# thu-ml/zhusuan

Hardware: NVIDIA B200
Metric: leapfrog-steps*chains/sec (higher is better)
Workload: dtype f32

## Files before the change

include/zsb200.h:

```cpp
#ifndef ZSB200_H_
#define ZSB200_H_
#include <stddef.h>
#include <stdint.h>

#ifdef __cplusplus
extern "C" {
#endif

#define ZSB_OK 0
#define ZSB_ERR_INVALID (-1)
#define ZSB_ERR_CUDA (-2)
#define ZSB_ERR_UNSUPPORTED (-3)

int zsb_version(void);
int zsb_last_error(char* buf, size_t n);
int zsb_device_count(void);
int zsb_stream_sync(void* stream);
int zsb_random_set_device_epoch(const uint32_t* epoch);
int zsb_random_bump_epoch(uint32_t* epoch, uint32_t by, void* stream);

enum {
  ZSB_HMC_STATE_T = 0, ZSB_HMC_STATE_STEP_SIZE = 1, ZSB_HMC_STATE_TUNER_STEP = 2,
  ZSB_HMC_STATE_LOG_EPS_BAR = 3, ZSB_HMC_STATE_H_BAR = 4, ZSB_HMC_STATE_MU = 5,
  ZSB_HMC_STATE_EWMV_T = 6, ZSB_HMC_STATE_EPS_USED = 7, ZSB_HMC_STATE_ACC_MEAN = 8,
// ... 153 lines not shown
                               int64_t D, int impl, void* stream);
int zsb_hmc_dense_tc_config(int bk);
int zsb_hmc_dense_split_lo_f32(const float* q, float* lo, int64_t n, void* stream);
int zsb_hmc_dense_h16_prepare_f32(const float* q, void* planes, float* scales, int64_t n,
                                  void* stream);
int zsb_hmc_dense_leapfrog_h16_f32(const float* q_cur, const void* q_cur_planes, float* q_next,
                                   void* q_next_planes, const float* p_in, float* p_out,
                                   const void* P_h16, const void* P_l16, const float* scales,
                                   const float* bvec, const float* mu, const float* mass,
                                   const float* state, float p_scale, float* lp_part,
                                   float* k_part, int64_t chains, int64_t D, void* stream);
int zsb_hmc_dense_h16i_prepare_f32(const float* q, float* scales, int64_t n, void* stream);
int zsb_hmc_dense_leapfrog_h16i_f32(const float* q_cur, float* q_next, const float* p_in,
                                    float* p_out, const void* P_h16, const void* P_l16,
                                    float* scales, int pass_index, const float* bvec,
                                    const float* mu, const float* mass, const float* state,
                                    float p_scale, float* lp_part, float* k_part, int64_t chains,
                                    int64_t D, void* stream);
int zsb_hmc_dense_trajectory_h16_f32(const float* q0, const void* planes0, float* qa,
                                     void* planes_a, float* qb, void* planes_b, const float* p0,
                                     float* pw, const void* P_h16, const void* P_l16,
                                     const float* scales, const float* bvec, const float* mu,
                                     const float* mass, const float* state, float* lp0_part,
                                     float* lp1_part, float* k_part, int64_t chains, int64_t D,
                                     int n_leapfrogs, void* stream);
int zsb_hmc_dense_resident_flags(int64_t chains);
int zsb_hmc_dense_resident_group(int64_t D);
int zsb_hmc_dense_resident_h16_f32(void* planes0, void* planes1, const float* p0, float* pw,
                                   const void* P_h16, const void* P_l16, const float* scales,
                                   const float* bvec, const float* mu, const float* mass,
                                   const float* state, float* lp0_part, float* lp1_part,
                                   float* k_part, int32_t* flags, int64_t chains, int64_t D,
                                   int n_leapfrogs, void* stream);
int zsb_hmc_dense_select_planes_f32(float* q, const void* planes, const float* scales,
                                    const int32_t* accept, int64_t chains, int64_t D,
                                    void* stream);
int zsb_hmc_dense_finish_f32(const float* lp_part, const float* k_part, int ntiles, int64_t chains,
                             float const_term, float* lp_out, float* k_out, void* stream);

int zsb_sample_categorical_i32(const float* logits, int64_t logit_rows, int64_t rows,
                               int64_t n_categories, int64_t n_samples, const float* u,
                               uint64_t seed, uint32_t iter, int32_t* out, void* stream);
int zsb_sample_dirichlet_f32(const float* alpha, int64_t alpha_rows, int64_t n_rows,
                             int64_t n_categories, const float* gammas, uint64_t seed,
                             uint32_t iter, float* out, void* stream);
int zsb_sample_gamma_f32(const float* alpha, int64_t alpha_rows, const float* beta,
                         int64_t beta_rows, int64_t n_rows, int64_t row_len, uint64_t seed,
                         uint32_t iter, float* out, void* stream);
int zsb_sample_base_noise_f32(int kind, float* out, int64_t n, uint64_t seed, uint32_t iter,
                              void* stream);
int zsb_sample_count_i32(int kind, const float* param, int64_t param_n, int64_t n_experiments,
                         const float* u, uint64_t seed, uint32_t iter, int32_t* out, int64_t n,
                         void* stream);

int zsb_lntm_phi_t_f32(const float* beta, int64_t n_topics, int64_t n_vocab, float* phi_t,
                       void* stream);
int zsb_lntm_logjoint_f32(const float* eta, const float* eta_mean, const float* eta_logstd,
                          const float* phi_t, const int64_t* doc_ptr, const int32_t* word_idx,
                          const float* word_cnt, float* lp_out, float* grad_out, int64_t chains,
                          int64_t docs, int64_t n_topics, void* stream);

int zsb_sgmcmc_parts(void);
int zsb_sgmcmc_sgld_f32(float* q, const float* g, const float* noise, float lr, int64_t chains,
                        int64_t row_len, uint64_t seed, uint32_t iter, int64_t row0,
                        void* stream);
int zsb_sgmcmc_psgld_f32(float* q, float* aux, const float* g, const float* noise, float lr,
// ... 36 lines not shown
```

zhusuan_b200/csrc/hmc_dense.cu:

```cuda
#include "common.cuh"

namespace {

constexpr int BM = 128, BN = 128, BK = 16;
constexpr int APAD = 4;


__global__ void __launch_bounds__(256, 2)
dense_leapfrog_simt_kernel(const float* __restrict__ q_cur, float* __restrict__ q_next,
                           const float* __restrict__ p_in, float* __restrict__ p_out,
                           const float* __restrict__ P, const float* __restrict__ bvec,
                           const float* __restrict__ mu, const float* __restrict__ mass,
                           const float* __restrict__ state, float p_scale,
                           float* __restrict__ lp_part, float* __restrict__ k_part,
                           int64_t chains, int D) {
  __shared__ __align__(16) float As[2][BK][BM + APAD];
  __shared__ __align__(16) float Bs[2][BK][BN];

  const int tid = threadIdx.x;
  const int tx = tid & 15, ty = tid >> 4;
  const int64_t m0 = (int64_t)blockIdx.y * BM;
  const int n0 = blockIdx.x * BN;

  const int a_row = tid >> 2;
// ... 136 lines not shown
int zsb_dense_split_lo_launch(const float* q, float* lo, int64_t n, cudaStream_t st);
int zsb_dense_tc_ntiles(int D);
int zsb_dense_tc_set_bk(int bk);
int zsb_dense_leapfrog_h16_launch(const float* q_cur, const void* q_cur_planes, float* q_next,
                                  void* q_next_planes, const float* p_in, float* p_out,
                                  const void* P_h16, const void* P_l16, const float* scales,
                                  const float* bvec, const float* mu, const float* mass,
                                  const float* state, float p_scale, float* lp_part, float* k_part,
                                  int64_t chains, int D, cudaStream_t st);
int zsb_dense_h16_prepare_launch(const float* q, void* planes, float* scales, int64_t n,
                                 cudaStream_t st);
int zsb_dense_leapfrog_h16i_launch(const float* q_cur, float* q_next, const float* p_in,
                                   float* p_out, const void* P_h16, const void* P_l16,
                                   float* scales, int pass_index, const float* bvec,
                                   const float* mu, const float* mass, const float* state,
                                   float p_scale, float* lp_part, float* k_part, int64_t chains,
                                   int D, cudaStream_t st);
int zsb_dense_h16i_prepare_launch(const float* q, float* scales, int64_t n, cudaStream_t st);
int zsb_dense_traj_h16_launch(const float* q0, const void* planes0, float* qa, void* planes_a,
                              float* qb, void* planes_b, const float* p0, float* pw,
                              const void* P_h16, const void* P_l16, const float* scales,
                              const float* bvec, const float* mu, const float* mass,
                              const float* state, float* lp0_part, float* lp1_part,
                              float* k_part, int64_t chains, int D, int L, cudaStream_t st);
int zsb_dense_res_h16_launch(void* planes0, void* planes1, const float* p0, float* pw,
                             const void* P_h16, const void* P_l16, const float* scales,
                             const float* bvec, const float* mu, const float* mass,
                             const float* state, float* lp0_part, float* lp1_part, float* k_part,
                             int* flags, int64_t chains, int D, int L, cudaStream_t st);
int zsb_dense_select_planes_launch(float* q, const void* planes, const float* scales,
                                   const int32_t* accept, int64_t chains, int64_t D,
                                   cudaStream_t st);
int zsb_dense_res_group_blocks(int D);

extern "C" {

int zsb_hmc_dense_ntiles(int64_t D, int impl) {
  if (impl == 1) return zsb_dense_tc_ntiles((int)D);
  return (int)zsb_ceil_div(D, BN);
}

int zsb_hmc_dense_leapfrog_f32(const float* q_cur, const float* q_cur_lo, float* q_next,
                               float* q_next_lo, const float* p_in, float* p_out,
                               const float* P, const float* P_lo, const float* bvec,
                               const float* mu, const float* mass, const float* state,
                               float p_scale, float* lp_part, float* k_part, int64_t chains,
                               int64_t D, int impl, void* stream) {
  ZSB_REQUIRE(q_cur && p_in && p_out && P && mass && state, "zsb_hmc_dense_leapfrog_f32: null arg");
  ZSB_REQUIRE(chains > 0 && D > 0 && D % BK == 0 && D <= (1 << 20),
              "zsb_hmc_dense_leapfrog_f32: D must be a positive multiple of 16");
  ZSB_REQUIRE(q_next != q_cur, "zsb_hmc_dense_leapfrog_f32: q_next must not alias q_cur");
  cudaStream_t st = (cudaStream_t)stream;
  if (impl == 1) {
    ZSB_REQUIRE(P_lo && q_cur_lo, "zsb_hmc_dense_leapfrog_f32: impl 1 needs the P_lo / q_lo splits");
    return zsb_dense_leapfrog_tc_launch(q_cur, q_cur_lo, q_next, q_next_lo, p_in, p_out, P, P_lo,
                                        bvec, mu, mass, state, p_scale, lp_part, k_part, chains,
                                        (int)D, st);
  }
  ZSB_REQUIRE(impl == 0, "zsb_hmc_dense_leapfrog_f32: unknown impl %d", impl);
  dim3 grid((unsigned)zsb_ceil_div(D, BN), (unsigned)zsb_ceil_div(chains, BM));
  dense_leapfrog_simt_kernel<<<grid, 256, 0, st>>>(q_cur, q_next, p_in, p_out, P, bvec, mu, mass,
                                                   state, p_scale, lp_part, k_part, chains, (int)D);
  return zsb_check_launch("hmc_dense_leapfrog_simt");
}

int zsb_hmc_dense_tc_config(int bk) {
// ... 45 lines not shown
}

int zsb_hmc_dense_trajectory_h16_f32(const float* q0, const void* planes0, float* qa,
                                     void* planes_a, float* qb, void* planes_b, const float* p0,
                                     float* pw, const void* P_h16, const void* P_l16,
                                     const float* scales, const float* bvec, const float* mu,
                                     const float* mass, const float* state, float* lp0_part,
                                     float* lp1_part, float* k_part, int64_t chains, int64_t D,
                                     int n_leapfrogs, void* stream) {
  ZSB_REQUIRE(q0 && planes0 && qa && planes_a && qb && planes_b && p0 && pw && P_h16 && P_l16 &&
                  scales && mass && state && lp0_part && lp1_part && k_part,
              "zsb_hmc_dense_trajectory_h16_f32: null arg");
  return zsb_dense_traj_h16_launch(q0, planes0, qa, planes_a, qb, planes_b, p0, pw, P_h16, P_l16,
                                   scales, bvec, mu, mass, state, lp0_part, lp1_part, k_part,
                                   chains, (int)D, n_leapfrogs, (cudaStream_t)stream);
}

int zsb_hmc_dense_resident_flags(int64_t chains) { return 2 * (int)zsb_ceil_div(chains, 256); }
int zsb_hmc_dense_resident_group(int64_t D) { return zsb_dense_res_group_blocks((int)D); }
int zsb_hmc_dense_resident_h16_f32(void* planes0, void* planes1, const float* p0, float* pw,
                                   const void* P_h16, const void* P_l16, const float* scales,
                                   const float* bvec, const float* mu, const float* mass,
                                   const float* state, float* lp0_part, float* lp1_part,
                                   float* k_part, int32_t* flags, int64_t chains, int64_t D,
                                   int n_leapfrogs, void* stream) {
  ZSB_REQUIRE(planes0 && planes1 && p0 && pw && P_h16 && P_l16 && scales && mass && state &&
                  lp0_part && lp1_part && k_part && flags,
              "zsb_hmc_dense_resident_h16_f32: null arg");
  ZSB_REQUIRE(p0 != pw, "zsb_hmc_dense_resident_h16_f32: aliased buffers");
  return zsb_dense_res_h16_launch(planes0, planes1, p0, pw, P_h16, P_l16, scales, bvec, mu, mass,
                                  state, lp0_part, lp1_part, k_part, flags, chains, (int)D,
                                  n_leapfrogs, (cudaStream_t)stream);
}
int zsb_hmc_dense_select_planes_f32(float* q, const void* planes, const float* scales,
                                    const int32_t* accept, int64_t chains, int64_t D,
                                    void* stream) {
  ZSB_REQUIRE(q && planes && scales && accept && chains > 0 && D > 0 && D % 2 == 0,
              "zsb_hmc_dense_select_planes_f32: bad args");
  return zsb_dense_select_planes_launch(q, planes, scales, accept, chains, D,
                                        (cudaStream_t)stream);
}

int zsb_hmc_dense_finish_f32(const float* lp_part, const float* k_part, int ntiles, int64_t chains,
                             float const_term, float* lp_out, float* k_out, void* stream) {
  ZSB_REQUIRE(chains > 0 && ntiles > 0, "zsb_hmc_dense_finish_f32: bad sizes");
  int64_t blocks = zsb_ceil_div(chains, 256);
  if (blocks > ZSB_NUM_SMS * 8) blocks = ZSB_NUM_SMS * 8;
  dense_finish_kernel<<<(unsigned)blocks, 256, 0, (cudaStream_t)stream>>>(
      lp_part, k_part, ntiles, chains, const_term, lp_out, k_out);
  return zsb_check_launch("hmc_dense_finish");
}

}
```

zhusuan_b200/csrc/hmc_dense_res.cu:

```cuda
#include "tc_common.cuh"

namespace {

using CR = Cfg2<32>;

struct ResMaps {
  CUtensorMap p_hi, p_lo;
  CUtensorMap q_hi[2], q_lo[2];
};

__device__ __forceinline__ int flag_load_acquire(const int* f) {
  int v;
  asm volatile("ld.acquire.gpu.global.s32 %0, [%1];" : "=r"(v) : "l"(f) : "memory");
  return v;
}
__device__ __forceinline__ void flag_add_release(int* f, int v) {
  asm volatile("red.release.gpu.global.add.s32 [%0], %1;" ::"l"(f), "r"(v) : "memory");
}
__device__ __forceinline__ void flag_wait(const int* f, int target) {
  if (flag_load_acquire(f) >= target) return;
  const long long t0 = clock64();
  while (flag_load_acquire(f) < target) {
    __nanosleep(64);
    if (clock64() - t0 > WAIT_TIMEOUT_CYCLES) {
      printf("zsb dense_res: flag wait timeout (block %d thread %d target %d have %d)\n",
             blockIdx.x, threadIdx.x, target, flag_load_acquire(f));
      __trap();
    }
  }
}

__device__ __forceinline__ void tma_load_2d_2sm_mc(uint32_t dst, const CUtensorMap* map,
                                                   uint32_t bar, int c0, int c1, uint16_t mask) {
  asm volatile(
      "cp.async.bulk.tensor.2d.cta_group::2.shared::cluster.global.mbarrier::complete_tx::bytes"
      ".multicast::cluster [%0], [%1, {%4, %5}], [%2], %3;"
      ::"r"(dst), "l"(map), "r"(bar & PEER_BIT_MASK), "h"(mask), "r"(c0), "r"(c1)
      : "memory");
}
__device__ __forceinline__ void umma_commit_mask(uint32_t bar, uint16_t mask) {
  asm volatile(
      "tcgen05.commit.cta_group::2.mbarrier::arrive::one.shared::cluster.multicast::cluster.b64"
      " [%0], %1;"
      ::"r"(bar), "h"(mask) : "memory");
}

struct ResEpi {
  const __half* __restrict__ hi_cur; const __half* __restrict__ lo_cur;
  __half* __restrict__ hi_nxt; __half* __restrict__ lo_nxt;
  const float* __restrict__ p_in; float* __restrict__ p_out;
  float* __restrict__ lp_part; float* __restrict__ k_part;
  int64_t chains; int D;
  float sq, inv_sq, acc_scale;
};

template <int MODE, int NEXT, int DC>
__device__ __forceinline__ void epilogue_planes(const ResEpi& a, uint32_t trow, int n, bool n_ok,
                                                bool parts_ok, int64_t c0, int64_t part_row,
                                                int lane, float s2, float eps_over_m_sq,
                                                float inv_m, float b_n, float mu_n, bool skip) {
  constexpr int NCOL = BN / 2;
  const uint32_t D = DC ? (uint32_t)DC : (uint32_t)a.D;
  const int64_t chains = a.chains;
  const bool warp_n_ok = __all_sync(0xffffffffu, n_ok);
  const bool fast_tile = warp_n_ok && (c0 + NCOL <= chains) && !skip;
  const int64_t off_t = c0 * (int64_t)D + n;
  const float* __restrict__ pin0 = a.p_in + off_t;
  float* __restrict__ po0 = a.p_out + off_t;
  const unsigned short* __restrict__ hc0 =
      reinterpret_cast<const unsigned short*>(a.hi_cur) + off_t;
  const unsigned short* __restrict__ lc0 =
      reinterpret_cast<const unsigned short*>(a.lo_cur) + off_t;
  __half* __restrict__ hn0 = NEXT ? a.hi_nxt + off_t : nullptr;
  __half* __restrict__ ln0 = NEXT ? a.lo_nxt + off_t : nullptr;

  auto element = [&](float acc, float p, uint32_t hl, float& pn, float& lpv, float& kv,
                     __half& hh, __half& ll) {
    const float Q = __half2float(__ushort_as_half((unsigned short)(hl & 0xFFFFu))) +
                    __half2float(__ushort_as_half((unsigned short)(hl >> 16)));
    const float g = b_n - a.acc_scale * acc;
    pn = fmaf(s2, g, p);
    if (MODE >= 1) lpv = (Q * a.inv_sq - mu_n) * g;
    if (MODE >= 2) kv = pn * pn * inv_m;
    if (NEXT) {
      const float Qn = fmaf(eps_over_m_sq, pn, Q);
      hh = __float2half_rn(Qn);
      ll = __float2half_rn(Qn - __half2float(hh));
    }
  };

  if (fast_tile) {
    auto load = [&](float* pe, uint32_t* he, int c) {
      const size_t cb = (size_t)c * D;
#pragma unroll
      for (int j = 0; j < 16; ++j) {
        pe[j] = __ldcg(pin0 + cb + (uint32_t)j * D);
        const uint32_t h = __ldcg(hc0 + cb + (uint32_t)j * D);
        const uint32_t l = __ldcg(lc0 + cb + (uint32_t)j * D);
        he[j] = h | (l << 16);
      }
    };
    auto compute = [&](const uint32_t* v, const float* pe, const uint32_t* he, int c) {
      const size_t cb = (size_t)c * D;
      float lpv[MODE >= 1 ? 16 : 1], kv[MODE >= 2 ? 16 : 1];
#pragma unroll
      for (int j = 0; j < 16; ++j) {
        float pn, lp1 = 0.f, k1 = 0.f;
        __half hh, ll;
        element(__uint_as_float(v[j]), pe[j], he[j], pn, lp1, k1, hh, ll);
        po0[cb + (uint32_t)j * D] = pn;
        if (MODE >= 1) lpv[j] = lp1;
        if (MODE >= 2) kv[j] = k1;
        if (NEXT) {
          hn0[cb + (uint32_t)j * D] = hh;
          ln0[cb + (uint32_t)j * D] = ll;
        }
      }
      if (MODE >= 1) {
        const float sum = warp_transpose_sum16(lpv, lane);
        if (lane < 16) a.lp_part[part_row + c0 + c + lane] = sum;
      }
      if (MODE >= 2) {
        const float sum = warp_transpose_sum16(kv, lane);
        if (lane < 16) a.k_part[part_row + c0 + c + lane] = sum;
      }
    };
    float pa[16], pb[16];
    uint32_t ha[16], hb[16], va[16], vb[16];
    load(pa, ha, 0);
    tmem_ld16(trow, va);
#pragma unroll 1
    for (int c = 0; c < NCOL; c += 32) {
      load(pb, hb, c + 16);
      tmem_ld_wait();
      tmem_ld16(trow + (uint32_t)(c + 16), vb);
      compute(va, pa, ha, c);
      if (c + 32 < NCOL) load(pa, ha, c + 32);
      tmem_ld_wait();
      if (c + 32 < NCOL) tmem_ld16(trow + (uint32_t)(c + 32), va);
      compute(vb, pb, hb, c + 16);
    }
  } else {
#pragma unroll 1
    for (int c = 0; c < NCOL; c += 16) {
      uint32_t v[16];
      tmem_ld16(trow + (uint32_t)c, v);
      tmem_ld_wait();
      const int64_t cbase = c0 + c;
      if (cbase < chains && !skip) {
        const size_t cb = (size_t)c * D;
        float lpv[MODE >= 1 ? 16 : 1], kv[MODE >= 2 ? 16 : 1];
#pragma unroll
        for (int j = 0; j < 16; ++j) {
          const bool ok = n_ok && cbase + j < chains;
          float p = 0.f;
          uint32_t hl = 0u;
          if (ok) {
            p = __ldcg(pin0 + cb + (uint32_t)j * D);
            hl = (uint32_t)__ldcg(hc0 + cb + (uint32_t)j * D) |
                 ((uint32_t)__ldcg(lc0 + cb + (uint32_t)j * D) << 16);
          }
          float pn, lp1 = 0.f, k1 = 0.f;
          __half hh, ll;
          element(__uint_as_float(v[j]), p, hl, pn, lp1, k1, hh, ll);
          if (MODE >= 1) lpv[j] = ok ? lp1 : 0.f;
          if (MODE >= 2) kv[j] = ok ? k1 : 0.f;
          if (ok) {
            po0[cb + (uint32_t)j * D] = pn;
            if (NEXT) {
              hn0[cb + (uint32_t)j * D] = hh;
              ln0[cb + (uint32_t)j * D] = ll;
            }
          }
        }
        if (MODE >= 1) {
          const float sum = warp_transpose_sum16(lpv, lane);
          if (parts_ok && lane < 16 && cbase + lane < chains)
            a.lp_part[part_row + cbase + lane] = sum;
        }
        if (MODE >= 2) {
          const float sum = warp_transpose_sum16(kv, lane);
          if (parts_ok && lane < 16 && cbase + lane < chains)
            a.k_part[part_row + cbase + lane] = sum;
        }
      }
    }
  }
}

template <int DC, int MC>
__global__ void __launch_bounds__(NUM_THREADS, 1)
dense_res_kernel(const __grid_constant__ ResMaps maps, __half* __restrict__ planes0,
                 __half* __restrict__ planes1, const float* __restrict__ p0,
                 float* __restrict__ pw, const float* __restrict__ bvec,
                 const float* __restrict__ mu, const float* __restrict__ mass,
                 const float* __restrict__ state, float* __restrict__ lp0_part,
                 float* __restrict__ lp1_part, float* __restrict__ k_part, int64_t chains,
                 int D_rt, int L, const float* __restrict__ scales, int* __restrict__ flags,
                 int group_blocks, int dbg, int inplace) {
  using C = CR;
  const int D = DC ? DC : D_rt;
  extern __shared__ uint8_t smem_raw[];
  const uint32_t smem_base = (smem_u32(smem_raw) + 1023u) & ~1023u;
  const uint32_t bars = smem_base + C::STAGES * C::STAGE;
  const uint32_t full_bar = bars;
  const uint32_t empty_bar = bars + 8 * C::STAGES;
  const uint32_t tfull_bar = bars + 16 * C::STAGES;
  const uint32_t tempty_bar = bars + 16 * C::STAGES + 16;
  const uint32_t tmem_slot = bars + 16 * C::STAGES + 32;
  uint32_t* tmem_slot_ptr =
      reinterpret_cast<uint32_t*>(smem_raw + (tmem_slot - smem_u32(smem_raw)));

  const int warp = __shfl_sync(0xffffffffu, (int)(threadIdx.x >> 5), 0);
  const int lane = threadIdx.x & 31;
  const uint32_t crank = cluster_ctarank();
  const uint32_t rank = crank & 1u;
  const uint32_t pidx = crank >> 1;
  const uint32_t leader_rank = crank & ~1u;
  const bool leader = rank == 0;
  const uint16_t pair_mask = (uint16_t)(3u << leader_rank);
  const int n_blk = (D + BM - 1) / BM;
  const int n_pair = (n_blk + 1) / 2;
  const int64_t c_blk = (chains + BN - 1) / BN;
  constexpr int CL = MC ? 4 : 2;
  const int64_t my = blockIdx.x / CL, n_clusters = gridDim.x / CL;
  const int n_kb = D / 64;
  const int flag_per_pass = n_pair * 2 * NUM_EPI_WARPS;

  if (threadIdx.x == 0) {
    for (int s = 0; s < C::STAGES; ++s) {
      mbar_init(full_bar + 8 * s, 1);
      mbar_init(empty_bar + 8 * s, MC ? 2 : 1);
    }
    for (int a = 0; a < 2; ++a) {
      mbar_init(tfull_bar + 8 * a, 1);
      mbar_init(tempty_bar + 8 * a, 2 * 32 * NUM_EPI_WARPS);
    }
    asm volatile("fence.mbarrier_init.release.cluster;" ::: "memory");
  }
  if (warp == 1) {
    asm volatile("tcgen05.alloc.cta_group::2.sync.aligned.shared::cta.b32 [%0], %1;"
                 ::"r"(tmem_slot), "n"(TMEM_COLS) : "memory");
    asm volatile("tcgen05.relinquish_alloc_permit.cta_group::2.sync.aligned;" ::: "memory");
  }
  tc_fence_before();
  cluster_sync_all();
  tc_fence_after();
  const uint32_t tmem_base = *tmem_slot_ptr;

#define ZSB_RES_UNITS(gb) (MC ? (((gb) + 1) / 2) * n_pair : (gb) * n_pair)
#define ZSB_RES_BLOCK(g0, u) ((g0) + (MC ? 2 * ((u) / n_pair) + (int64_t)pidx : (u) / n_pair))

  if (warp == 0) {
    if (lane == 0) {
      asm volatile("prefetch.tensormap [%0];" ::"l"(&maps.p_hi) : "memory");
      asm volatile("prefetch.tensormap [%0];" ::"l"(&maps.p_lo) : "memory");
      int stage = 0;
      uint32_t phase = 0;
      for (int64_t g0 = 0; g0 < c_blk; g0 += group_blocks) {
        const int64_t gb = (c_blk - g0 < group_blocks) ? (c_blk - g0) : group_blocks;
        const int64_t units = ZSB_RES_UNITS(gb);
        for (int i = 0; i <= L; ++i) {
          const int buf = inplace ? 0 : (i & 1);
          for (int64_t u = my; u < units; u += n_clusters) {
            const int64_t cb = ZSB_RES_BLOCK(g0, u);
            const bool valid = cb < g0 + gb;
            const int n0 = ((int)(u % n_pair) * 2 + (int)rank) * BM;
            const int c0 = (int)(cb * BN) + (int)rank * (BN / 2);
            if (i > 0 && valid && !(dbg & 4)) {
              flag_wait(flags + cb, i * flag_per_pass);
              asm volatile("fence.proxy.async;" ::: "memory");
            }
            for (int kb = 0; kb < n_kb; ++kb) {
              mbar_wait(empty_bar + 8 * stage, phase ^ 1);
              const uint32_t fb = full_bar + 8 * stage;
              const uint32_t sa = smem_base + stage * C::STAGE;
              if (leader) mbar_expect_tx(fb, 2 * C::STAGE);
              if (MC) {
                const uint16_t mm = (uint16_t)(5u << rank);
                const uint32_t ho = pidx * (uint32_t)(C::A_TILE / 2);
                tma_load_2d_2sm_mc(sa + ho, &maps.p_hi, fb, kb * 64, n0 + (int)pidx * (BM / 2),
                                   mm);
                tma_load_2d_2sm_mc(sa + C::A_TILE + ho, &maps.p_lo, fb, kb * 64,
                                   n0 + (int)pidx * (BM / 2), mm);
              } else {
                tma_load_2d_2sm(sa, &maps.p_hi, fb, kb * 64, n0);
                tma_load_2d_2sm(sa + C::A_TILE, &maps.p_lo, fb, kb * 64, n0);
              }
              tma_load_2d_2sm(sa + 2 * C::A_TILE, &maps.q_hi[buf], fb, kb * 64, c0);
              tma_load_2d_2sm(sa + 2 * C::A_TILE + C::B_TILE, &maps.q_lo[buf], fb, kb * 64, c0);
              if (++stage == C::STAGES) { stage = 0; phase ^= 1; }
            }
          }
        }
      }
    }
  } else if (warp == 1) {
    if (leader && lane == 0) {
      const uint32_t idesc = make_idesc_2sm_f16();
      int stage = 0;
      uint32_t phase = 0;
      int acc = 0;
      uint32_t acc_phase = 0;
      for (int64_t g0 = 0; g0 < c_blk; g0 += group_blocks) {
        const int64_t gb = (c_blk - g0 < group_blocks) ? (c_blk - g0) : group_blocks;
        const int64_t units = ZSB_RES_UNITS(gb);
        for (int i = 0; i <= L; ++i) {
          for (int64_t u = my; u < units; u += n_clusters) {
            mbar_wait(tempty_bar + 8 * acc, acc_phase ^ 1);
            tc_fence_after();
            const uint32_t d_tmem = tmem_base + (uint32_t)(acc * BN);
            for (int kb = 0; kb < n_kb; ++kb) {
              mbar_wait(full_bar + 8 * stage, phase);
              tc_fence_after();
              const uint32_t sa = smem_base + stage * C::STAGE;
              const uint64_t a_hi = make_smem_desc<32>(sa);
              const uint64_t a_lo = make_smem_desc<32>(sa + C::A_TILE);
              const uint64_t b_hi = make_smem_desc<32>(sa + 2 * C::A_TILE);
              const uint64_t b_lo = make_smem_desc<32>(sa + 2 * C::A_TILE + C::B_TILE);
#pragma unroll
              for (int k = 0; k < 4; ++k) {
                const uint64_t ko = (uint64_t)((k * 32) >> 4);
                const uint32_t first = (kb | k) != 0 ? 1u : 0u;
                if (dbg & 2) {
                  umma_f16_2sm(d_tmem, a_hi + ko, b_hi + ko, idesc, first);
                } else {
                  umma_f16_2sm(d_tmem, a_lo + ko, b_hi + ko, idesc, first);
                  umma_f16_2sm(d_tmem, a_hi + ko, b_lo + ko, idesc, 1u);
                  umma_f16_2sm(d_tmem, a_hi + ko, b_hi + ko, idesc, 1u);
                }
              }
              umma_commit_mask(empty_bar + 8 * stage, MC ? (uint16_t)0xF : pair_mask);
              if (++stage == C::STAGES) { stage = 0; phase ^= 1; }
            }
            umma_commit_mask(tfull_bar + 8 * acc, pair_mask);
            if (++acc == 2) { acc = 0; acc_phase ^= 1; }
          }
        }
      }
    }
  } else {
    const int quarter = warp & 3;
    const int half = (warp - 2) >> 2;
    const float eps = state[ZSB_ST_EPS_USED];
    const float sq = scales[0];
    const int64_t plane = chains * (int64_t)D;
    __half* pl[2] = {planes0, inplace ? planes0 : planes1};
    int acc = 0;
    uint32_t acc_phase = 0;
    for (int64_t g0 = 0; g0 < c_blk; g0 += group_blocks) {
      const int64_t gb = (c_blk - g0 < group_blocks) ? (c_blk - g0) : group_blocks;
      const int64_t units = ZSB_RES_UNITS(gb);
      for (int i = 0; i <= L; ++i) {
        const bool last = i == L;
        const float s2 = mul(eps, (i > 0 && !last) ? 1.f : 0.5f);
        const int buf = i & 1;
        for (int64_t u = my; u < units; u += n_clusters) {
          const int64_t cb = ZSB_RES_BLOCK(g0, u);
          const bool valid = cb < g0 + gb;
          const int nb = (int)(u % n_pair) * 2 + (int)rank;
          const int n = nb * BM + quarter * 32 + lane;
          const int64_t c0 = cb * BN + half * (BN / 2);
          const bool n_ok = n < D;
          const float m_n = n_ok ? mass[n] : 1.f;
          const float eps_over_m_sq = mul(fdiv(eps, m_n), sq);
          const float inv_m = fdiv(1.f, m_n);
          const float b_n = (n_ok && bvec) ? bvec[n] : 0.f;
          const float mu_n = (n_ok && mu) ? mu[n] : 0.f;
          mbar_wait(tfull_bar + 8 * acc, acc_phase);
          tc_fence_after();
          if (inplace && valid && !last) {
            int* mma_done = flags + c_blk;
            if (leader && warp == 2 && lane == 0) flag_add_release(mma_done + cb, 1);
            if (lane == 0) flag_wait(mma_done + cb, (i + 1) * n_pair);
            __syncwarp();
          }
          const uint32_t trow = tmem_base + ((uint32_t)(quarter * 32) << 16) +
                                (uint32_t)(acc * BN + half * (BN / 2));
          const int64_t part_row = (int64_t)(nb * 4 + quarter) * chains;
          const ResEpi ea{pl[buf], pl[buf] + plane, pl[buf ^ 1], pl[buf ^ 1] + plane,
                          i == 0 ? p0 : pw, pw, i == 0 ? lp0_part : lp1_part, k_part,
                          chains, D, sq, fdiv(1.f, sq), scales[1]};
          const bool skip = (dbg & 1) != 0 || !valid;
          if (last)
            epilogue_planes<2, 0, DC>(ea, trow, n, n_ok, nb < n_blk, c0, part_row, lane, s2,
                                      eps_over_m_sq, inv_m, b_n, mu_n, skip);
          else if (i == 0)
            epilogue_planes<1, 1, DC>(ea, trow, n, n_ok, nb < n_blk, c0, part_row, lane, s2,
                                      eps_over_m_sq, inv_m, b_n, mu_n, skip);
          else
            epilogue_planes<0, 1, DC>(ea, trow, n, n_ok, nb < n_blk, c0, part_row, lane, s2,
                                      eps_over_m_sq, inv_m, b_n, mu_n, skip);
          tc_fence_before();
          if (leader) mbar_arrive(tempty_bar + 8 * acc);
          else mbar_arrive_remote(tempty_bar + 8 * acc, leader_rank);
          if (!last && valid) {
            __threadfence();
            asm volatile("fence.proxy.async;" ::: "memory");
            __syncwarp();
            if (lane == 0) flag_add_release(flags + cb, 1);
          }
          if (++acc == 2) { acc = 0; acc_phase ^= 1; }
        }
      }
    }
  }

#undef ZSB_RES_UNITS
#undef ZSB_RES_BLOCK
  tc_fence_before();
  cluster_sync_all();
  if (warp == 1) {
    tc_fence_after();
    asm volatile("tcgen05.dealloc.cta_group::2.sync.aligned.b32 %0, %1;"
                 ::"r"(tmem_base), "n"(TMEM_COLS) : "memory");
  }
}

__global__ void __launch_bounds__(256) select_planes_kernel(float* __restrict__ q,
                                                            const __half* __restrict__ planes,
                                                            const float* __restrict__ scales,
                                                            const int32_t* __restrict__ accept,
                                                            int64_t chains, int64_t D) {
  const float inv_sq = 1.f / scales[0];
  const int lane = threadIdx.x & 31;
  const int n8 = (int)(D >> 3);
  const int64_t wstride = (int64_t)gridDim.x * 8;
  for (int64_t c = (int64_t)blockIdx.x * 8 + (threadIdx.x >> 5); c < chains; c += wstride) {
    if (!accept[c]) continue;
    const uint4* __restrict__ hi = reinterpret_cast<const uint4*>(planes + c * D);
    const uint4* __restrict__ lo = reinterpret_cast<const uint4*>(planes + (chains + c) * D);
    float4* __restrict__ qr = reinterpret_cast<float4*>(q + c * D);
    for (int i0 = lane; i0 < n8; i0 += 128) {
      uint4 h[4], l[4];
#pragma unroll
      for (int u = 0; u < 4; ++u) {
        const int i = i0 + 32 * u;
        if (i < n8) { h[u] = __ldcs(hi + i); l[u] = __ldcs(lo + i); }
      }
#pragma unroll
      for (int u = 0; u < 4; ++u) {
        const int i = i0 + 32 * u;
        if (i < n8) {
          const uint32_t hw[4] = {h[u].x, h[u].y, h[u].z, h[u].w};
          const uint32_t lw[4] = {l[u].x, l[u].y, l[u].z, l[u].w};
          float o[8];
#pragma unroll
          for (int k = 0; k < 4; ++k) {
            const float2 hf = __half22float2(*reinterpret_cast<const __half2*>(&hw[k]));
            const float2 lf = __half22float2(*reinterpret_cast<const __half2*>(&lw[k]));
            o[2 * k] = (hf.x + lf.x) * inv_sq;
            o[2 * k + 1] = (hf.y + lf.y) * inv_sq;
          }
          qr[2 * i] = make_float4(o[0], o[1], o[2], o[3]);
          qr[2 * i + 1] = make_float4(o[4], o[5], o[6], o[7]);
        }
      }
    }
  }
}

template <int DC, int MC>
cudaError_t res_prepare() {
  static const cudaError_t e = cudaFuncSetAttribute(
      dense_res_kernel<DC, MC>, cudaFuncAttributeMaxDynamicSharedMemorySize, CR::SMEM);
  return e;
}

int res_mc_env() {
  static const int mc = getenv("ZSB_RES_MC") ? atoi(getenv("ZSB_RES_MC")) : -1;
  return mc;
}

template <int DC, int MC>
int res_max_clusters(int cl, int sms) {
  cudaLaunchConfig_t cfg = {};
  cfg.gridDim = dim3((unsigned)(cl * (sms / cl)));
  cfg.blockDim = dim3(NUM_THREADS);
  cfg.dynamicSmemBytes = CR::SMEM;
  cudaLaunchAttribute at[1];
  at[0].id = cudaLaunchAttributeClusterDimension;
  at[0].val.clusterDim.x = (unsigned)cl; at[0].val.clusterDim.y = 1; at[0].val.clusterDim.z = 1;
  cfg.attrs = at; cfg.numAttrs = 1;
  int n = 0;
  if (cudaOccupancyMaxActiveClusters(&n, dense_res_kernel<DC, MC>, &cfg) != cudaSuccess || n < 1) {
    cudaGetLastError();
    n = sms / cl;
  }
  return n;
}

}

void res_choose(int D, int64_t chains, int* mc_out, int* group_out) {
  static const int env_group = getenv("ZSB_RES_GROUP") ? atoi(getenv("ZSB_RES_GROUP")) : 0;
  int dev = 0, sms = ZSB_NUM_SMS;
  cudaGetDevice(&dev);
  cudaDeviceGetAttribute(&sms, cudaDevAttrMultiProcessorCount, dev);
  const int n_pair = ((D + BM - 1) / BM + 1) / 2;
  const int64_t c_blk = (chains + BN - 1) / BN;
  int mc = res_mc_env();
  int max_cl4 = 0;
  if (mc != 0 && res_prepare<0, 1>() == cudaSuccess) {
    static const int cached = res_max_clusters<0, 1>(4, sms);
    max_cl4 = cached;
  }
  if (mc < 0) mc = (max_cl4 > 0 && c_blk * n_pair >= 4 * (int64_t)max_cl4) ? 1 : 0;
  if (mc && max_cl4 <= 0) mc = 0;
  int g = mc ? 2 * ((2 * max_cl4) / n_pair) : (2 * (sms / 2)) / n_pair;
  if (env_group > 0) g = env_group;
  if (g < 1) g = 1;
  if (getenv("ZSB_RES_VERBOSE"))
    fprintf(stderr, "zsb dense_res: multicast %d (%d co-resident clusters of 4), group = %d blocks\n",
            mc, max_cl4, g);
  *mc_out = mc;
  *group_out = g;
}

// ... 5 lines not shown

int zsb_dense_res_h16_launch(void* planes0, void* planes1, const float* p0, float* pw,
                             const void* P_h16, const void* P_l16, const float* scales,
                             const float* bvec, const float* mu, const float* mass,
                             const float* state, float* lp0_part, float* lp1_part, float* k_part,
                             int* flags, int64_t chains, int D, int L, cudaStream_t st) {
  if (D % 64 != 0 || D < 64 || L < 1 || chains <= 0 || chains >= (1LL << 31)) {
    zsb_set_error("dense_res: needs D %% 64 == 0, n_leapfrogs >= 1");
    return ZSB_ERR_INVALID;
  }
  ResMaps m;
  int rc;
  int mc = 0, group = 1;
  res_choose(D, chains, &mc, &group);
  const uint32_t a_rows = mc ? BM / 2 : BM;
  if ((rc = make_map(&m.p_hi, P_h16, (uint64_t)D, (uint64_t)D, a_rows, 32, 1))) return rc;
  if ((rc = make_map(&m.p_lo, P_l16, (uint64_t)D, (uint64_t)D, a_rows, 32, 1))) return rc;
  const __half* pl[2] = {reinterpret_cast<const __half*>(planes0),
                         reinterpret_cast<const __half*>(planes1)};
  for (int b = 0; b < 2; ++b) {
    if ((rc = make_map(&m.q_hi[b], pl[b], (uint64_t)chains, (uint64_t)D, BN / 2, 32, 1)))
      return rc;
    if ((rc = make_map(&m.q_lo[b], pl[b] + chains * D, (uint64_t)chains, (uint64_t)D, BN / 2, 32,
                       1)))
      return rc;
  }
  int dev = 0, sms = ZSB_NUM_SMS;
  cudaGetDevice(&dev);
  cudaDeviceGetAttribute(&sms, cudaDevAttrMultiProcessorCount, dev);
  const int n_pair = ((D + BM - 1) / BM + 1) / 2;
  const int64_t c_blk = (chains + BN - 1) / BN;
  if (group > c_blk) group = (int)c_blk;
  static const int env_dbg = getenv("ZSB_RES_DBG") ? atoi(getenv("ZSB_RES_DBG")) : 0;
  const int inplace = planes0 == planes1 ? 1 : 0;
  cudaError_t e = cudaMemsetAsync(flags, 0, sizeof(int) * (size_t)c_blk * 2, st);
  if (e != cudaSuccess) {
    zsb_set_error("dense_res: cudaMemsetAsync: %s", cudaGetErrorString(e));
    return ZSB_ERR_CUDA;
  }
  const int cl = mc ? 4 : 2;
  cudaError_t prep = cudaSuccess, le = cudaSuccess;
  __half* pl0 = reinterpret_cast<__half*>(planes0);
  __half* pl1 = reinterpret_cast<__half*>(planes1);
  int Di = D, Li = L, dbg = env_dbg;
#define ZSB_RES_LAUNCH(DC, MCV)                                                                 \
  do {                                                                                          \
    prep = res_prepare<DC, MCV>();                                                              \
    if (prep != cudaSuccess) break;                                                             \
    static const int max_cl = res_max_clusters<DC, MCV>(cl, sms);                               \
    int64_t clusters = max_cl;                                                                  \
    const int64_t units = MCV ? (int64_t)((group + 1) / 2) * n_pair : (int64_t)group * n_pair;  \
    if (units < clusters) clusters = units;                                                     \
    cudaLaunchConfig_t cfg = {};                                                                \
    cfg.gridDim = dim3((unsigned)(cl * clusters));                                              \
    cfg.blockDim = dim3(NUM_THREADS);                                                           \
    cfg.dynamicSmemBytes = CR::SMEM;                                                            \
    cfg.stream = st;                                                                            \
    cudaLaunchAttribute at[1];                                                                  \
    at[0].id = cudaLaunchAttributeClusterDimension;                                             \
    at[0].val.clusterDim.x = (unsigned)cl; at[0].val.clusterDim.y = 1;                          \
    at[0].val.clusterDim.z = 1;                                                                 \
    cfg.attrs = at; cfg.numAttrs = 1;                                                           \
    le = cudaLaunchKernelEx(&cfg, dense_res_kernel<DC, MCV>, m, pl0, pl1, p0, pw, bvec, mu,     \
                            mass, state, lp0_part, lp1_part, k_part, chains, Di, Li, scales,    \
                            flags, group, dbg, inplace);                                        \
  } while (0)
  if (mc) { if (D == 1024) ZSB_RES_LAUNCH(1024, 1); else ZSB_RES_LAUNCH(0, 1); }
  else { if (D == 1024) ZSB_RES_LAUNCH(1024, 0); else ZSB_RES_LAUNCH(0, 0); }
#undef ZSB_RES_LAUNCH
  if (prep != cudaSuccess || le != cudaSuccess) {
    zsb_set_error("dense_res: launch setup: %s",
                  cudaGetErrorString(prep != cudaSuccess ? prep : le));
    return ZSB_ERR_CUDA;
  }
  return zsb_check_launch("hmc_dense_resident");
}

int zsb_dense_select_planes_launch(float* q, const void* planes, const float* scales,
                                   const int32_t* accept, int64_t chains, int64_t D,
                                   cudaStream_t st) {
  ZSB_REQUIRE(D % 8 == 0, "zsb_dense_select_planes: D must be a multiple of 8");
  int64_t blocks = zsb_ceil_div(chains, 8);
  if (blocks > ZSB_NUM_SMS * 16) blocks = ZSB_NUM_SMS * 16;
  if (blocks < 1) blocks = 1;
  select_planes_kernel<<<(unsigned)blocks, 256, 0, st>>>(
      q, reinterpret_cast<const __half*>(planes), scales, accept, chains, D);
  return zsb_check_launch("hmc_select_planes");
}
```

Measured before the change: 156.4 million.

## Add L2 cache-policy hints to resident HMC kernel and simplify TMEM epilogue pipeline

Attaches L2 eviction-policy hints to the TMA loads of the P and q planes: evict_last while they are still reused across leapfrog passes, evict_normal on the final pass. The epilogue's global loads use evict_unchanged, and its stores use evict_last for next-state planes or evict_first otherwise. The aim is to keep the precision matrix and state planes resident in L2 across passes. It also drops the double-buffered TMEM load in the epilogue for a single buffer loaded just before each compute, which saves registers but gives less overlap. An env-gated profiling template variant with clock64 counters and a readout API is added as well; it is off by default.

```diff
diff --git a/include/zsb200.h b/include/zsb200.h
--- a/include/zsb200.h
+++ b/include/zsb200.h
@@ -209,6 +209,7 @@
                                    const float* state, float* lp0_part, float* lp1_part,
                                    float* k_part, int32_t* flags, int64_t chains, int64_t D,
                                    int n_leapfrogs, void* stream);
+int zsb_hmc_dense_resident_prof( int64_t* counters, int n_slots, int reset);
 int zsb_hmc_dense_select_planes_f32(float* q, const void* planes, const float* scales,
                                     const int32_t* accept, int64_t chains, int64_t D,
                                     void* stream);
diff --git a/zhusuan_b200/csrc/hmc_dense.cu b/zhusuan_b200/csrc/hmc_dense.cu
--- a/zhusuan_b200/csrc/hmc_dense.cu
+++ b/zhusuan_b200/csrc/hmc_dense.cu
@@ -192,6 +192,7 @@
                                    const int32_t* accept, int64_t chains, int64_t D,
                                    cudaStream_t st);
 int zsb_dense_res_group_blocks(int D);
+int dense_res_prof_read(int64_t* out, int n_slots, int reset);
 
 extern "C" {
 
@@ -303,6 +304,10 @@
                                   state, lp0_part, lp1_part, k_part, flags, chains, (int)D,
                                   n_leapfrogs, (cudaStream_t)stream);
 }
+int zsb_hmc_dense_resident_prof(int64_t* counters, int n_slots, int reset) {
+  ZSB_REQUIRE(counters && n_slots > 0, "zsb_hmc_dense_resident_prof: bad args");
+  return dense_res_prof_read(counters, n_slots, reset);
+}
 int zsb_hmc_dense_select_planes_f32(float* q, const void* planes, const float* scales,
                                     const int32_t* accept, int64_t chains, int64_t D,
                                     void* stream) {
diff --git a/zhusuan_b200/csrc/hmc_dense_res.cu b/zhusuan_b200/csrc/hmc_dense_res.cu
--- a/zhusuan_b200/csrc/hmc_dense_res.cu
+++ b/zhusuan_b200/csrc/hmc_dense_res.cu
@@ -8,6 +8,59 @@
   CUtensorMap p_hi, p_lo;
   CUtensorMap q_hi[2], q_lo[2];
 };
+
+enum ResProfSlot {
+  RP_LAUNCHES, RP_PROD_TOTAL, RP_PROD_EMPTY, RP_PROD_FLAGS, RP_MMA_TOTAL, RP_MMA_FULL,
+  RP_MMA_TEMPTY, RP_EPI_TOTAL, RP_EPI_TFULL, RP_EPI_MMADONE, RP_EPI_BODY, RP_EPI_PUBLISH,
+  RP_SLOTS = 16
+};
+__device__ unsigned long long g_res_prof[RP_SLOTS];
+
+__device__ __forceinline__ uint64_t l2_evict_last() {
+  uint64_t p;
+  asm volatile("createpolicy.fractional.L2::evict_last.b64 %0, 1.0;" : "=l"(p));
+  return p;
+}
+__device__ __forceinline__ uint64_t l2_evict_normal() {
+  uint64_t p;
+  asm volatile("createpolicy.fractional.L2::evict_normal.b64 %0, 1.0;" : "=l"(p));
+  return p;
+}
+__device__ __forceinline__ uint64_t l2_evict_unchanged() {
+  uint64_t p;
+  asm volatile("createpolicy.fractional.L2::evict_unchanged.b64 %0, 1.0;" : "=l"(p));
+  return p;
+}
+__device__ __forceinline__ uint64_t l2_evict_first() {
+  uint64_t p;
+  asm volatile("createpolicy.fractional.L2::evict_first.b64 %0, 1.0;" : "=l"(p));
+  return p;
+}
+__device__ __forceinline__ float ld_cg_pol(const float* a, uint64_t pol) {
+  float v;
+  asm volatile("ld.global.cg.L2::cache_hint.f32 %0, [%1], %2;" : "=f"(v) : "l"(a), "l"(pol));
+  return v;
+}
+__device__ __forceinline__ unsigned short ld_cg_pol(const unsigned short* a, uint64_t pol) {
+  unsigned short v;
+  asm volatile("ld.global.cg.L2::cache_hint.u16 %0, [%1], %2;" : "=h"(v) : "l"(a), "l"(pol));
+  return v;
+}
+__device__ __forceinline__ void st_pol(float* a, float v, uint64_t pol) {
+  asm volatile("st.global.L2::cache_hint.f32 [%0], %1, %2;" ::"l"(a), "f"(v), "l"(pol) : "memory");
+}
+__device__ __forceinline__ void st_pol(__half* a, __half v, uint64_t pol) {
+  asm volatile("st.global.L2::cache_hint.b16 [%0], %1, %2;"
+               ::"l"(a), "h"(__half_as_ushort(v)), "l"(pol) : "memory");
+}
+__device__ __forceinline__ void tma_load_2d_2sm_pol(uint32_t dst, const CUtensorMap* map,
+                                                    uint32_t bar, int c0, int c1, uint64_t pol) {
+  asm volatile(
+      "cp.async.bulk.tensor.2d.cta_group::2.shared::cluster.global.mbarrier::complete_tx::bytes"
+      ".L2::cache_hint [%0], [%1, {%3, %4}], [%2], %5;"
+      ::"r"(dst), "l"(map), "r"(bar & PEER_BIT_MASK), "r"(c0), "r"(c1), "l"(pol)
+      : "memory");
+}
 
 __device__ __forceinline__ int flag_load_acquire(const int* f) {
   int v;
@@ -31,11 +84,12 @@
 }
 
 __device__ __forceinline__ void tma_load_2d_2sm_mc(uint32_t dst, const CUtensorMap* map,
-                                                   uint32_t bar, int c0, int c1, uint16_t mask) {
+                                                   uint32_t bar, int c0, int c1, uint16_t mask,
+                                                   uint64_t pol) {
   asm volatile(
       "cp.async.bulk.tensor.2d.cta_group::2.shared::cluster.global.mbarrier::complete_tx::bytes"
-      ".multicast::cluster [%0], [%1, {%4, %5}], [%2], %3;"
-      ::"r"(dst), "l"(map), "r"(bar & PEER_BIT_MASK), "h"(mask), "r"(c0), "r"(c1)
+      ".multicast::cluster.L2::cache_hint [%0], [%1, {%4, %5}], [%2], %3, %6;"
+      ::"r"(dst), "l"(map), "r"(bar & PEER_BIT_MASK), "h"(mask), "r"(c0), "r"(c1), "l"(pol)
       : "memory");
 }
 __device__ __forceinline__ void umma_commit_mask(uint32_t bar, uint16_t mask) {
@@ -60,6 +114,8 @@
                                                 int lane, float s2, float eps_over_m_sq,
                                                 float inv_m, float b_n, float mu_n, bool skip) {
   constexpr int NCOL = BN / 2;
+  const uint64_t pol_ld = l2_evict_unchanged();
+  const uint64_t pol_st = NEXT ? l2_evict_last() : l2_evict_first();
   const uint32_t D = DC ? (uint32_t)DC : (uint32_t)a.D;
   const int64_t chains = a.chains;
   const bool warp_n_ok = __all_sync(0xffffffffu, n_ok);
@@ -94,9 +150,9 @@
       const size_t cb = (size_t)c * D;
 #pragma unroll
       for (int j = 0; j < 16; ++j) {
-        pe[j] = __ldcg(pin0 + cb + (uint32_t)j * D);
-        const uint32_t h = __ldcg(hc0 + cb + (uint32_t)j * D);
-        const uint32_t l = __ldcg(lc0 + cb + (uint32_t)j * D);
+        pe[j] = ld_cg_pol(pin0 + cb + (uint32_t)j * D, pol_ld);
+        const uint32_t h = ld_cg_pol(hc0 + cb + (uint32_t)j * D, pol_ld);
+        const uint32_t l = ld_cg_pol(lc0 + cb + (uint32_t)j * D, pol_ld);
         he[j] = h | (l << 16);
       }
     };
@@ -108,12 +164,12 @@
         float pn, lp1 = 0.f, k1 = 0.f;
         __half hh, ll;
         element(__uint_as_float(v[j]), pe[j], he[j], pn, lp1, k1, hh, ll);
-        po0[cb + (uint32_t)j * D] = pn;
+        st_pol(po0 + cb + (uint32_t)j * D, pn, pol_st);
         if (MODE >= 1) lpv[j] = lp1;
         if (MODE >= 2) kv[j] = k1;
         if (NEXT) {
-          hn0[cb + (uint32_t)j * D] = hh;
-          ln0[cb + (uint32_t)j * D] = ll;
+          st_pol(hn0 + cb + (uint32_t)j * D, hh, pol_st);
+          st_pol(ln0 + cb + (uint32_t)j * D, ll, pol_st);
         }
       }
       if (MODE >= 1) {
@@ -126,19 +182,18 @@
       }
     };
     float pa[16], pb[16];
-    uint32_t ha[16], hb[16], va[16], vb[16];
+    uint32_t ha[16], hb[16], v[16];
     load(pa, ha, 0);
-    tmem_ld16(trow, va);
 #pragma unroll 1
     for (int c = 0; c < NCOL; c += 32) {
       load(pb, hb, c + 16);
+      tmem_ld16(trow + (uint32_t)c, v);
       tmem_ld_wait();
-      tmem_ld16(trow + (uint32_t)(c + 16), vb);
-      compute(va, pa, ha, c);
+      compute(v, pa, ha, c);
       if (c + 32 < NCOL) load(pa, ha, c + 32);
+      tmem_ld16(trow + (uint32_t)(c + 16), v);
       tmem_ld_wait();
-      if (c + 32 < NCOL) tmem_ld16(trow + (uint32_t)(c + 32), va);
-      compute(vb, pb, hb, c + 16);
+      compute(v, pb, hb, c + 16);
     }
   } else {
 #pragma unroll 1
@@ -156,9 +211,9 @@
           float p = 0.f;
           uint32_t hl = 0u;
           if (ok) {
-            p = __ldcg(pin0 + cb + (uint32_t)j * D);
-            hl = (uint32_t)__ldcg(hc0 + cb + (uint32_t)j * D) |
-                 ((uint32_t)__ldcg(lc0 + cb + (uint32_t)j * D) << 16);
+            p = ld_cg_pol(pin0 + cb + (uint32_t)j * D, pol_ld);
+            hl = (uint32_t)ld_cg_pol(hc0 + cb + (uint32_t)j * D, pol_ld) |
+                 ((uint32_t)ld_cg_pol(lc0 + cb + (uint32_t)j * D, pol_ld) << 16);
           }
           float pn, lp1 = 0.f, k1 = 0.f;
           __half hh, ll;
@@ -166,10 +221,10 @@
           if (MODE >= 1) lpv[j] = ok ? lp1 : 0.f;
           if (MODE >= 2) kv[j] = ok ? k1 : 0.f;
           if (ok) {
-            po0[cb + (uint32_t)j * D] = pn;
+            st_pol(po0 + cb + (uint32_t)j * D, pn, pol_st);
             if (NEXT) {
-              hn0[cb + (uint32_t)j * D] = hh;
-              ln0[cb + (uint32_t)j * D] = ll;
+              st_pol(hn0 + cb + (uint32_t)j * D, hh, pol_st);
+              st_pol(ln0 + cb + (uint32_t)j * D, ll, pol_st);
             }
           }
         }
@@ -188,7 +243,7 @@
   }
 }
 
-template <int DC, int MC>
+template <int DC, int MC, int PROF>
 __global__ void __launch_bounds__(NUM_THREADS, 1)
 dense_res_kernel(const __grid_constant__ ResMaps maps, __half* __restrict__ planes0,
                  __half* __restrict__ planes1, const float* __restrict__ p0,
@@ -255,6 +310,9 @@
     if (lane == 0) {
       asm volatile("prefetch.tensormap [%0];" ::"l"(&maps.p_hi) : "memory");
       asm volatile("prefetch.tensormap [%0];" ::"l"(&maps.p_lo) : "memory");
+      const uint64_t pol_keep = l2_evict_last(), pol_done = l2_evict_normal();
+      long long t_start = 0, t_empty = 0, t_flags = 0;
+      if constexpr (PROF) t_start = clock64();
       int stage = 0;
       uint32_t phase = 0;
       for (int64_t g0 = 0; g0 < c_blk; g0 += group_blocks) {
@@ -262,17 +320,24 @@
         const int64_t units = ZSB_RES_UNITS(gb);
         for (int i = 0; i <= L; ++i) {
           const int buf = inplace ? 0 : (i & 1);
+          const uint64_t pol = (i == L || (!inplace && i == L - 1)) ? pol_done : pol_keep;
           for (int64_t u = my; u < units; u += n_clusters) {
             const int64_t cb = ZSB_RES_BLOCK(g0, u);
             const bool valid = cb < g0 + gb;
             const int n0 = ((int)(u % n_pair) * 2 + (int)rank) * BM;
             const int c0 = (int)(cb * BN) + (int)rank * (BN / 2);
             if (i > 0 && valid && !(dbg & 4)) {
+              long long t0 = 0;
+              if constexpr (PROF) t0 = clock64();
               flag_wait(flags + cb, i * flag_per_pass);
+              if constexpr (PROF) t_flags += clock64() - t0;
               asm volatile("fence.proxy.async;" ::: "memory");
             }
             for (int kb = 0; kb < n_kb; ++kb) {
+              long long t0 = 0;
+              if constexpr (PROF) t0 = clock64();
               mbar_wait(empty_bar + 8 * stage, phase ^ 1);
+              if constexpr (PROF) t_empty += clock64() - t0;
               const uint32_t fb = full_bar + 8 * stage;
               const uint32_t sa = smem_base + stage * C::STAGE;
               if (leader) mbar_expect_tx(fb, 2 * C::STAGE);
@@ -280,19 +345,26 @@
                 const uint16_t mm = (uint16_t)(5u << rank);
                 const uint32_t ho = pidx * (uint32_t)(C::A_TILE / 2);
                 tma_load_2d_2sm_mc(sa + ho, &maps.p_hi, fb, kb * 64, n0 + (int)pidx * (BM / 2),
-                                   mm);
+                                   mm, pol);
                 tma_load_2d_2sm_mc(sa + C::A_TILE + ho, &maps.p_lo, fb, kb * 64,
-                                   n0 + (int)pidx * (BM / 2), mm);
+                                   n0 + (int)pidx * (BM / 2), mm, pol);
               } else {
-                tma_load_2d_2sm(sa, &maps.p_hi, fb, kb * 64, n0);
-                tma_load_2d_2sm(sa + C::A_TILE, &maps.p_lo, fb, kb * 64, n0);
+                tma_load_2d_2sm_pol(sa, &maps.p_hi, fb, kb * 64, n0, pol);
+                tma_load_2d_2sm_pol(sa + C::A_TILE, &maps.p_lo, fb, kb * 64, n0, pol);
               }
-              tma_load_2d_2sm(sa + 2 * C::A_TILE, &maps.q_hi[buf], fb, kb * 64, c0);
-              tma_load_2d_2sm(sa + 2 * C::A_TILE + C::B_TILE, &maps.q_lo[buf], fb, kb * 64, c0);
+              tma_load_2d_2sm_pol(sa + 2 * C::A_TILE, &maps.q_hi[buf], fb, kb * 64, c0, pol);
+              tma_load_2d_2sm_pol(sa + 2 * C::A_TILE + C::B_TILE, &maps.q_lo[buf], fb, kb * 64, c0,
+                                  pol);
               if (++stage == C::STAGES) { stage = 0; phase ^= 1; }
             }
           }
         }
+      }
+      if constexpr (PROF) {
+        atomicAdd(&g_res_prof[RP_PROD_TOTAL], (unsigned long long)(clock64() - t_start));
+        atomicAdd(&g_res_prof[RP_PROD_EMPTY], (unsigned long long)t_empty);
+        atomicAdd(&g_res_prof[RP_PROD_FLAGS], (unsigned long long)t_flags);
+        if (blockIdx.x == 0) atomicAdd(&g_res_prof[RP_LAUNCHES], 1ull);
       }
     }
   } else if (warp == 1) {
@@ -302,16 +374,23 @@
       uint32_t phase = 0;
       int acc = 0;
       uint32_t acc_phase = 0;
+      long long t_start = 0, t_full = 0, t_tempty = 0;
+      if constexpr (PROF) t_start = clock64();
       for (int64_t g0 = 0; g0 < c_blk; g0 += group_blocks) {
         const int64_t gb = (c_blk - g0 < group_blocks) ? (c_blk - g0) : group_blocks;
         const int64_t units = ZSB_RES_UNITS(gb);
         for (int i = 0; i <= L; ++i) {
           for (int64_t u = my; u < units; u += n_clusters) {
+            long long t0 = 0;
+            if constexpr (PROF) t0 = clock64();
             mbar_wait(tempty_bar + 8 * acc, acc_phase ^ 1);
+            if constexpr (PROF) t_tempty += clock64() - t0;
             tc_fence_after();
             const uint32_t d_tmem = tmem_base + (uint32_t)(acc * BN);
             for (int kb = 0; kb < n_kb; ++kb) {
+              if constexpr (PROF) t0 = clock64();
               mbar_wait(full_bar + 8 * stage, phase);
+              if constexpr (PROF) t_full += clock64() - t0;
               tc_fence_after();
               const uint32_t sa = smem_base + stage * C::STAGE;
               const uint64_t a_hi = make_smem_desc<32>(sa);
@@ -338,6 +417,11 @@
           }
         }
       }
+      if constexpr (PROF) {
+        atomicAdd(&g_res_prof[RP_MMA_TOTAL], (unsigned long long)(clock64() - t_start));
+        atomicAdd(&g_res_prof[RP_MMA_FULL], (unsigned long long)t_full);
+        atomicAdd(&g_res_prof[RP_MMA_TEMPTY], (unsigned long long)t_tempty);
+      }
     }
   } else {
     const int quarter = warp & 3;
@@ -345,9 +429,11 @@
     const float eps = state[ZSB_ST_EPS_USED];
     const float sq = scales[0];
     const int64_t plane = chains * (int64_t)D;
-    __half* pl[2] = {planes0, inplace ? planes0 : planes1};
+    __half* const pl1 = inplace ? planes0 : planes1;
     int acc = 0;
     uint32_t acc_phase = 0;
+    long long t_start = 0, t_tfull = 0, t_mmadone = 0, t_body = 0, t_publish = 0, t0 = 0;
+    if constexpr (PROF) t_start = clock64();
     for (int64_t g0 = 0; g0 < c_blk; g0 += group_blocks) {
       const int64_t gb = (c_blk - g0 < group_blocks) ? (c_blk - g0) : group_blocks;
       const int64_t units = ZSB_RES_UNITS(gb);
@@ -367,21 +453,28 @@
           const float inv_m = fdiv(1.f, m_n);
           const float b_n = (n_ok && bvec) ? bvec[n] : 0.f;
           const float mu_n = (n_ok && mu) ? mu[n] : 0.f;
+          if constexpr (PROF) t0 = clock64();
           mbar_wait(tfull_bar + 8 * acc, acc_phase);
+          if constexpr (PROF) t_tfull += clock64() - t0;
           tc_fence_after();
           if (inplace && valid && !last) {
             int* mma_done = flags + c_blk;
             if (leader && warp == 2 && lane == 0) flag_add_release(mma_done + cb, 1);
+            if constexpr (PROF) t0 = clock64();
             if (lane == 0) flag_wait(mma_done + cb, (i + 1) * n_pair);
             __syncwarp();
+            if constexpr (PROF) t_mmadone += clock64() - t0;
           }
           const uint32_t trow = tmem_base + ((uint32_t)(quarter * 32) << 16) +
                                 (uint32_t)(acc * BN + half * (BN / 2));
           const int64_t part_row = (int64_t)(nb * 4 + quarter) * chains;
-          const ResEpi ea{pl[buf], pl[buf] + plane, pl[buf ^ 1], pl[buf ^ 1] + plane,
+          __half* const cur = buf ? pl1 : planes0;
+          __half* const nxt = buf ? planes0 : pl1;
+          const ResEpi ea{cur, cur + plane, nxt, nxt + plane,
                           i == 0 ? p0 : pw, pw, i == 0 ? lp0_part : lp1_part, k_part,
                           chains, D, sq, fdiv(1.f, sq), scales[1]};
           const bool skip = (dbg & 1) != 0 || !valid;
+          if constexpr (PROF) t0 = clock64();
           if (last)
             epilogue_planes<2, 0, DC>(ea, trow, n, n_ok, nb < n_blk, c0, part_row, lane, s2,
                                       eps_over_m_sq, inv_m, b_n, mu_n, skip);
@@ -394,14 +487,29 @@
           tc_fence_before();
           if (leader) mbar_arrive(tempty_bar + 8 * acc);
           else mbar_arrive_remote(tempty_bar + 8 * acc, leader_rank);
+          if constexpr (PROF) {
+            const long long t1 = clock64();
+            t_body += t1 - t0;
+            t0 = t1;
+          }
           if (!last && valid) {
             __threadfence();
             asm volatile("fence.proxy.async;" ::: "memory");
             __syncwarp();
             if (lane == 0) flag_add_release(flags + cb, 1);
           }
+          if constexpr (PROF) t_publish += clock64() - t0;
           if (++acc == 2) { acc = 0; acc_phase ^= 1; }
         }
+      }
+    }
+    if constexpr (PROF) {
+      if (lane == 0) {
+        atomicAdd(&g_res_prof[RP_EPI_TOTAL], (unsigned long long)(clock64() - t_start));
+        atomicAdd(&g_res_prof[RP_EPI_TFULL], (unsigned long long)t_tfull);
+        atomicAdd(&g_res_prof[RP_EPI_MMADONE], (unsigned long long)t_mmadone);
+        atomicAdd(&g_res_prof[RP_EPI_BODY], (unsigned long long)t_body);
+        atomicAdd(&g_res_prof[RP_EPI_PUBLISH], (unsigned long long)t_publish);
       }
     }
   }
@@ -460,10 +568,10 @@
   }
 }
 
-template <int DC, int MC>
+template <int DC, int MC, int PROF = 0>
 cudaError_t res_prepare() {
   static const cudaError_t e = cudaFuncSetAttribute(
-      dense_res_kernel<DC, MC>, cudaFuncAttributeMaxDynamicSharedMemorySize, CR::SMEM);
+      dense_res_kernel<DC, MC, PROF>, cudaFuncAttributeMaxDynamicSharedMemorySize, CR::SMEM);
   return e;
 }
 
@@ -472,7 +580,7 @@
   return mc;
 }
 
-template <int DC, int MC>
+template <int DC, int MC, int PROF = 0>
 int res_max_clusters(int cl, int sms) {
   cudaLaunchConfig_t cfg = {};
   cfg.gridDim = dim3((unsigned)(cl * (sms / cl)));
@@ -483,7 +591,8 @@
   at[0].val.clusterDim.x = (unsigned)cl; at[0].val.clusterDim.y = 1; at[0].val.clusterDim.z = 1;
   cfg.attrs = at; cfg.numAttrs = 1;
   int n = 0;
-  if (cudaOccupancyMaxActiveClusters(&n, dense_res_kernel<DC, MC>, &cfg) != cudaSuccess || n < 1) {
+  if (cudaOccupancyMaxActiveClusters(&n, dense_res_kernel<DC, MC, PROF>, &cfg) != cudaSuccess ||
+      n < 1) {
     cudaGetLastError();
     n = sms / cl;
   }
@@ -555,6 +664,7 @@
   const int64_t c_blk = (chains + BN - 1) / BN;
   if (group > c_blk) group = (int)c_blk;
   static const int env_dbg = getenv("ZSB_RES_DBG") ? atoi(getenv("ZSB_RES_DBG")) : 0;
+  static const bool env_prof = getenv("ZSB_RES_PROF") && atoi(getenv("ZSB_RES_PROF")) != 0;
   const int inplace = planes0 == planes1 ? 1 : 0;
   cudaError_t e = cudaMemsetAsync(flags, 0, sizeof(int) * (size_t)c_blk * 2, st);
   if (e != cudaSuccess) {
@@ -566,11 +676,11 @@
   __half* pl0 = reinterpret_cast<__half*>(planes0);
   __half* pl1 = reinterpret_cast<__half*>(planes1);
   int Di = D, Li = L, dbg = env_dbg;
-#define ZSB_RES_LAUNCH(DC, MCV)                                                                 \
+#define ZSB_RES_LAUNCH(DC, MCV, PROF)                                                           \
   do {                                                                                          \
-    prep = res_prepare<DC, MCV>();                                                              \
+    prep = res_prepare<DC, MCV, PROF>();                                                        \
     if (prep != cudaSuccess) break;                                                             \
-    static const int max_cl = res_max_clusters<DC, MCV>(cl, sms);                               \
+    static const int max_cl = res_max_clusters<DC, MCV, PROF>(cl, sms);                         \
     int64_t clusters = max_cl;                                                                  \
     const int64_t units = MCV ? (int64_t)((group + 1) / 2) * n_pair : (int64_t)group * n_pair;  \
     if (units < clusters) clusters = units;                                                     \
@@ -584,12 +694,17 @@
     at[0].val.clusterDim.x = (unsigned)cl; at[0].val.clusterDim.y = 1;                          \
     at[0].val.clusterDim.z = 1;                                                                 \
     cfg.attrs = at; cfg.numAttrs = 1;                                                           \
-    le = cudaLaunchKernelEx(&cfg, dense_res_kernel<DC, MCV>, m, pl0, pl1, p0, pw, bvec, mu,     \
-                            mass, state, lp0_part, lp1_part, k_part, chains, Di, Li, scales,    \
-                            flags, group, dbg, inplace);                                        \
+    le = cudaLaunchKernelEx(&cfg, dense_res_kernel<DC, MCV, PROF>, m, pl0, pl1, p0, pw, bvec,   \
+                            mu, mass, state, lp0_part, lp1_part, k_part, chains, Di, Li,        \
+                            scales, flags, group, dbg, inplace);                                \
   } while (0)
-  if (mc) { if (D == 1024) ZSB_RES_LAUNCH(1024, 1); else ZSB_RES_LAUNCH(0, 1); }
-  else { if (D == 1024) ZSB_RES_LAUNCH(1024, 0); else ZSB_RES_LAUNCH(0, 0); }
+  if (env_prof) {
+    if (mc) { if (D == 1024) ZSB_RES_LAUNCH(1024, 1, 1); else ZSB_RES_LAUNCH(0, 1, 1); }
+    else { if (D == 1024) ZSB_RES_LAUNCH(1024, 0, 1); else ZSB_RES_LAUNCH(0, 0, 1); }
+  } else {
+    if (mc) { if (D == 1024) ZSB_RES_LAUNCH(1024, 1, 0); else ZSB_RES_LAUNCH(0, 1, 0); }
+    else { if (D == 1024) ZSB_RES_LAUNCH(1024, 0, 0); else ZSB_RES_LAUNCH(0, 0, 0); }
+  }
 #undef ZSB_RES_LAUNCH
   if (prep != cudaSuccess || le != cudaSuccess) {
     zsb_set_error("dense_res: launch setup: %s",
@@ -597,6 +712,22 @@
     return ZSB_ERR_CUDA;
   }
   return zsb_check_launch("hmc_dense_resident");
+}
+
+int dense_res_prof_read(int64_t* out, int n_slots, int reset) {
+  if (n_slots > RP_SLOTS) n_slots = RP_SLOTS;
+  unsigned long long h[RP_SLOTS];
+  cudaError_t e = cudaMemcpyFromSymbol(h, g_res_prof, sizeof(h));
+  if (e == cudaSuccess && reset) {
+    const unsigned long long z[RP_SLOTS] = {};
+    e = cudaMemcpyToSymbol(g_res_prof, z, sizeof(z));
+  }
+  if (e != cudaSuccess) {
+    zsb_set_error("dense_res prof: %s", cudaGetErrorString(e));
+    return ZSB_ERR_CUDA;
+  }
+  for (int k = 0; k < n_slots; ++k) out[k] = (int64_t)h[k];
+  return ZSB_OK;
 }
 
 int zsb_dense_select_planes_launch(float* q, const void* planes, const float* scales,
```

Measured after the change: 161.8 million (median of 6 runs). 3.5% higher.
